# cliangyu/video-diffusion

Measured on AMD Instinct MI355X. Metric: denoise-steps/sec, higher is better.
Workload: dtype f32

## Files before the change

### include/vd_amd.h

```cpp
#ifndef VD_AMD_H
#define VD_AMD_H
#ifdef __cplusplus
extern "C" {
#endif

typedef struct vd_config {
    int image_size;
    int num_channels;
    int num_res_blocks;
    int num_heads;
    int T;
    int n_attention_ds;
    int attention_ds[8];
    int use_scale_shift_norm;
    int use_spatial_encoding;
    int use_frame_encoding;
    int enforce_position_invariance;
    int use_rpe_net;
    int allow_interactions_between_padding;
    float rp_alpha, rp_beta, rp_gamma;
    int time_embed_mult;
    int cond_emb_type;
    int learn_sigma;
} vd_config;
// ... 108 lines not shown
                  double* mse_out, void* stream);

int vd_window_begin(vd_engine* e, int B, int T, float* x, const float* obs_src, const float* obs_mask,
                    const float* latent_mask, const float* kinda_marg_mask, const long long* frame_indices,
                    int observed_frames, int sampler, int clip_denoised, float eta, unsigned long long seed,
                    unsigned long long offset, long long t_start, void* stream);
int vd_window_run(vd_engine* e, int n_steps, void* stream);
unsigned long long vd_window_generation(vd_engine* e);
int vd_window_graphs(vd_engine* e);

int vd_set_window_prefix_cache(vd_engine* e, int on);
int vd_window_prefix_frames(vd_engine* e);

int vd_set_window_suffix_skip(vd_engine* e, int on);
int vd_window_suffix_frames(vd_engine* e);

int vd_set_cfg_scale(vd_engine* e, float w);
float vd_cfg_scale(vd_engine* e);
int vd_op_cfg_combine(const float* out_c, const float* out_u, float w, long long n, float* out, void* stream);

int vd_set_guidance_rescale(vd_engine* e, float phi);
float vd_guidance_rescale(vd_engine* e);
int vd_set_dynamic_threshold(vd_engine* e, float p);
float vd_dynamic_threshold(vd_engine* e);
int vd_op_cfg_rescale(const float* out_c, const float* out_u, float w, const float* lat, int B, int T, long long frame_elems, float phi,
                      float* out, float* factor_out, void* stream);
int vd_op_dynamic_threshold(const float* x0, const float* lat, int B, int T, long long frame_elems, float p, float* out, float* s_out,
                            void* stream);

int vd_set_known_region(vd_engine* e, const float* known_src, const float* known_mask, const float* known_noise,
// ... 142 lines not shown
int vd_op_gn_bwd(const float* x0, const float* x1, int C0, int C, const float* affA, const float* affB, const float* mr,
                 const float* dy, int act, int nfr, int HW, const float* extra, float* dx0, int acc0, float* dx1, int acc1,
                 void* stream);
int vd_op_gn_temporal_bwd(const float* x, const float* gamma, const float* dy, int B, int T, int HW, int C, int accumulate,
                          float* dx, void* stream);
int vd_op_attn_temporal_bwd(const float* qkv, const float* Rk, const float* Rq, const float* Rv, const float* mask, int B,
                            int T, int HW, int C, int heads, int allow_pad, const float* dout, float* dqkv, void* stream);
int vd_op_attn_spatial_bwd(const float* qkv, int nfr, int L, int C, int heads, const float* dout, float* dqkv, void* stream);
int vd_op_out_conv_bwd(const float* deps, const float* w, int nfr, int H, int W, int C, int Cout, float* da, void* stream);
int vd_op_stem_col2im(const float* dcols, const float* obs, const float* lat, const float* km, int nfr, int H, int W,
                      int cond_mode, float* dx, void* stream);
int vd_op_sinus_embed(const float* t, int n, int dim, const float* freqs, float* out, void* stream);
int vd_op_frame_t(const long long* frame_indices, int B, int T, int center, float* tv, void* stream);
int vd_op_rpe_hidden(const float* te, int te_ld, const float* wbase, const long long* tab, const long long* frame_indices, int B, int T,
                     int C, float* E, int nz, long long zs_e, void* stream);
int vd_op_rpe_table(const float* table, const long long* frame_indices, int B, int T, int C, float alpha, float beta, float gamma,
                    float* R, void* stream);
int vd_op_posenc_add(const float* x, const float* P, const float* femb, int nfr, int HW, int C, float* y, void* stream);
int vd_op_assemble(const float* x, const float* obs_src, const float* obs_mask, const float* latent_mask, const float* kinda_marg_mask,
                   const float* t_model, int obs_t_mode, int B, int T, int H, int W, int Kpad, int cond_mode, const int* frame_list,
                   int n_list, int scalars_only, float* x_cols, float* t_frames, float* amask, void* stream);
int vd_op_move_rows(int scatter, const float* src, const int* list, int n, long long row_floats, float* dst, void* stream);
int vd_op_scatter_stats(const double* src, int split, int C, const int* list, int n, double* dst, void* stream);

typedef struct vd_lpips vd_lpips;
int vd_lpips_create(vd_lpips** out);
void vd_lpips_destroy(vd_lpips* h);
int vd_lpips_load_weight(vd_lpips* h, const char* name, const float* host, long long bytes);
long long vd_lpips_dim(int H, int W);
int vd_lpips_embed(vd_lpips* h, int N, int H, int W, const float* frames, float* out, void* stream);
// ... 28 lines not shown
```

### video-diffusion_amd/_lib.py

```python
import ctypes
import os
import subprocess

_HERE = os.path.dirname(os.path.abspath(__file__))
_CSRC = os.path.join(_HERE, "csrc")
SO_PATH = os.path.join(_HERE, "libvdamd.so")
SOURCES = ["igemm.hip", "conv_wino.hip", "conv_wino_r64.hip", "conv_wino_z128.hip", "gemm_frag.hip", "gemm_split.hip", "split_pack.hip", "norm.hip", "backward.hip", "attn_spatial.hip", "attn_temporal.hip", "attn_temporal_long.hip", "misc.hip", "guidance.hip", "known.hip", "measure.hip", "dps.hip", "ode_nll.hip", "engine.hip", "lpips.hip", "metrics.hip", "i3d.hip", "conv_cl.hip", "hallway.hip"]
HEADER = os.path.join(os.path.dirname(_HERE), "include", "vd_amd.h")
HEADERS = [os.path.join(_CSRC, "vd_common.h"), os.path.join(_CSRC, "wino_common.h"), os.path.join(_CSRC, "igemm_tile.h"), HEADER]
SOURCE_FLAGS = {"conv_wino_z128.hip": ["-mllvm", "-pragma-unroll-threshold=1000000"]}


def _toolchain():
    hipcc = os.environ.get("HIPCC", "/opt/rocm/bin/hipcc")
    flags = ["--offload-arch=gfx950", "-O3", "-std=c++17", "-fPIC", "-Wno-unused-value"] + \
        os.environ.get("VD_HIPCC_FLAGS", "").split()
    return hipcc, flags


def _sha(*parts):
    import hashlib
    h = hashlib.sha1()
    for p in parts:
        h.update(p if isinstance(p, bytes) else str(p).encode())
# ... 128 lines not shown
    "vd_dpmpp_2m_sde_sample": (_I, [_P, _I, _I, _P, _P, _P, _P, _P, _P, _P, _P, _I, _I, _P, _U, _U, _P, _P, _P, _P]),
    "vd_dpmpp_2m_sde_from_xstart": (_I, [_P, _I, _L, _P, _P, _P, _P, _I, _P, _U, _U, _P, _P, _P]),
    "vd_set_unipc_rows": (_I, [_P, _I, _P]),
    "vd_unipc_sample": (_I, [_P, _I, _I, _P, _P, _P, _P, _P, _P, _P, _P, _P, _P, _I, _I, _I, _P, _P, _P, _P, _P, _P, _P]),
    "vd_unipc_from_xstart": (_I, [_P, _I, _L, _P, _P, _P, _P, _P, _I, _P, _I, _P, _P, _P, _P, _P, _P]),
    "vd_p_mean_variance": (_I, [_P, _I, _I, _P, _P, _P, _P, _P, _P, _P, _I, _I, _P, _P, _P, _P]),
    "vd_vb_terms": (_I, [_P, _I, _I, _P, _P, _P, _P, _P, _I, _P, _P, _P, _P, _P, _P]),
    "vd_prior_bpd": (_I, [_P, _I, _I, _P, _P, _P, _P]),
    "vd_score_windows": (_I, [_P, _I, _I, _P, _P, _P, _P, _P, _P, _I, _U, _P, _P, _I, _P, _P]),
    "vd_op_eps_mse": (_I, [_P, _I, _I, _P, _P, _P, _I, _P, _U, _P, _P, _P, _P]),
    "vd_window_generation": (_U, [_P]),
    "vd_set_window_prefix_cache": (_I, [_P, _I]),
    "vd_window_prefix_frames": (_I, [_P]),
    "vd_set_window_suffix_skip": (_I, [_P, _I]),
    "vd_window_suffix_frames": (_I, [_P]),
    "vd_set_cfg_scale": (_I, [_P, _F]),
    "vd_cfg_scale": (_F, [_P]),
    "vd_op_cfg_combine": (_I, [_P, _P, _F, _L, _P, _P]),
    "vd_set_guidance_rescale": (_I, [_P, _F]),
    "vd_guidance_rescale": (_F, [_P]),
    "vd_set_dynamic_threshold": (_I, [_P, _F]),
    "vd_dynamic_threshold": (_F, [_P]),
    "vd_op_cfg_rescale": (_I, [_P, _P, _F, _P, _I, _I, _L, _F, _P, _P, _P]),
    "vd_op_dynamic_threshold": (_I, [_P, _P, _I, _I, _L, _F, _P, _P, _P]),
    "vd_set_known_region": (_I, [_P, _P, _P, _P, _U, _U]),
    "vd_known_region": (_I, [_P]),
    "vd_known_merge": (_I, [_P, _I, _I, _L, _P, _P, _P, _P, _P, _P, _U, _U, _P]),
    "vd_set_jump_rows": (_I, [_P, _I, _P, _P]),
    "vd_q_jump": (_I, [_P, _I, _I, _L, _P, _P, _P, _P, _U, _U, _P, _P]),
    "vd_window_jump": (_I, [_P, _I, _P]),
# ... 66 lines not shown
    "vd_igemm_variant_list": (_I, [ctypes.c_char_p, _I]),
    "vd_conv_wino_ksplit": (_I, [_I, _I, _I, _I]),
    "vd_op_conv_wino_split_k": (_I, [_P, _I, _I, _I, _I, _I, _P, _P, _P, _P, _I, _P, _I, _P, _I, _P]),
    "vd_op_linear_split_side": (_I, [_P, _P, _I, _I, _I, _I, _P, _P, _P, _P, _P, _P, _I, _P]),
    "vd_op_linear_batched": (_I, [_P, _I, _I, _I, _I, _P, _P, _P, _P]),
    "vd_op_out_conv": (_I, [_P, _P, _P, _P, _P, _I, _I, _I, _I, _I, _P, _P]),
    "vd_op_gn_bwd": (_I, [_P, _P, _I, _I, _P, _P, _P, _P, _I, _I, _I, _P, _P, _I, _P, _I, _P]),
    "vd_op_gn_temporal_bwd": (_I, [_P, _P, _P, _I, _I, _I, _I, _I, _P, _P]),
    "vd_op_attn_temporal_bwd": (_I, [_P, _P, _P, _P, _P, _I, _I, _I, _I, _I, _I, _P, _P, _P]),
    "vd_op_attn_spatial_bwd": (_I, [_P, _I, _I, _I, _I, _P, _P, _P]),
    "vd_op_out_conv_bwd": (_I, [_P, _P, _I, _I, _I, _I, _I, _P, _P]),
    "vd_op_stem_col2im": (_I, [_P, _P, _P, _P, _I, _I, _I, _I, _P, _P]),
    "vd_op_sinus_embed": (_I, [_P, _I, _I, _P, _P, _P]),
    "vd_op_frame_t": (_I, [_P, _I, _I, _I, _P, _P]),
    "vd_op_rpe_hidden": (_I, [_P, _I, _P, _P, _P, _I, _I, _I, _P, _I, _L, _P]),
    "vd_op_rpe_table": (_I, [_P, _P, _I, _I, _I, _F, _F, _F, _P, _P]),
    "vd_op_posenc_add": (_I, [_P, _P, _P, _I, _I, _I, _P, _P]),
    "vd_op_assemble": (_I, [_P, _P, _P, _P, _P, _P, _I, _I, _I, _I, _I, _I, _I, _P, _I, _I, _P, _P, _P, _P]),
    "vd_op_move_rows": (_I, [_I, _P, _P, _I, _L, _P, _P]),
    "vd_op_scatter_stats": (_I, [_P, _I, _I, _P, _I, _P, _P]),
    "vd_lpips_create": (_I, [ctypes.POINTER(_P)]),
    "vd_lpips_destroy": (None, [_P]),
    "vd_lpips_load_weight": (_I, [_P, ctypes.c_char_p, _P, _L]),
    "vd_lpips_dim": (_L, [_I, _I]),
    "vd_lpips_embed": (_I, [_P, _I, _I, _I, _P, _P, _P]),
    "vd_fps_select": (_I, [_I, _I, _L, _P, _I, _P, _I, _P, _P, _P]),
    "vd_frame_metrics": (_I, [_I, _I, _I, _I, _P, _P, _I, _D, _P, _P, _P]),
    "vd_pair_sqdist": (_I, [_I, _L, _P, _P, _P, _P]),
    "vd_i3d_create": (_I, [ctypes.POINTER(_P)]),
    "vd_i3d_destroy": (None, [_P]),
# ... 55 lines not shown
```

### video-diffusion_amd/csrc/engine.hip

```cpp
#include <cmath>
#include <cstring>
#include <unordered_map>
#include <vector>

#include "../../include/vd_amd.h"
#include "vd_common.h"

namespace vd {

thread_local std::string g_last_error;
void set_error(const std::string& msg) { g_last_error = msg; }

int launch_frame_t(const int64_t* fidx, int B, int T, int center, float* tv, hipStream_t s);

enum ParamKind { PK_RAW = 0, PK_CONV3, PK_STEM, PK_POSENC, PK_OUTCONV, PK_LINF, PK_CONV3W, PK_CONV3S,
                 PK_CONV3WU };

struct Param {
    std::string name;
    int nd = 0;
    long long shape[4] = {1, 1, 1, 1};
    size_t numel = 0;
    size_t packed = 0;
    size_t off = 0;
// ... 176 lines not shown
    int suf_blk = -2, suf_layer = -1;
    int p_posenc = -1, p_te0w, p_te0b, p_te2w, p_te2b, p_outgw, p_outgb, p_outw, p_outb;
    size_t film_w_off = 0, film_b_off = 0, te_w_off = 0, te_b_off = 0;
    int film_total = 0, te_total = 0;
    size_t packed_total = 0;
    float* wbuf = nullptr;
    bool wbuf_on_host = false;
    int put(void* dst, const void* src, size_t bytes) {
        if (wbuf_on_host) { std::memcpy(dst, src, bytes); return 0; }
        VD_HIP(hipMemcpy(dst, src, bytes, hipMemcpyHostToDevice));
        return 0;
    }
    struct RpeGroup { int C; std::vector<int> blocks; long long* d_hid = nullptr; long long* d_out = nullptr; };
    std::vector<RpeGroup> rpe_groups;
    std::vector<float*> rpe_R;
    int rpe_all(const float* te, const int64_t* fidx, int B, int T, hipStream_t st, Arena& ar);
    int rpe_tables();
    void rpe_group_blocks();
    float* d_freq_time = nullptr; int n_freq_time = 0;
    float* d_freq_frame = nullptr; int n_freq_frame = 0;
    float* d_tab = nullptr; int num_timesteps = 0;
    float* d_tmap = nullptr; float rescale = 1.f;
    float* d_w2m = nullptr;
    float* d_unipc = nullptr;
    float* d_jump = nullptr;
    char* ws = nullptr; size_t ws_cap = 0;
    bool ws_suf = false;
    int ws_B = 0, ws_T = 0; size_t ws_tail = 0;
    std::unordered_map<long long, size_t> ws_peaks;
    static size_t tm_bytes(int B) { return ((size_t)B * sizeof(float) + 255) & ~(size_t)255; }
    size_t out_floats(int B, int T) const { return (size_t)B * T * (cfg.learn_sigma ? 6 : 3) * cfg.image_size * cfg.image_size; }
// ... 664 lines not shown
            const RpeP* rp[3] = {&a.rq, &a.rk, &a.rv};
            for (int k = 0; k < 3; ++k) {
                const int z = 3 * (int)i + k;
                th[3 * z] = rp[k]->te_off; th[3 * z + 1] = (long long)params[rp[k]->dw].off; th[3 * z + 2] = (long long)params[rp[k]->db].off;
                to[2 * z] = (long long)params[rp[k]->ow].off; to[2 * z + 1] = (long long)params[rp[k]->ob].off;
            }
        }
        VD_HIP(hipMalloc(reinterpret_cast<void**>(&g.d_hid), th.size() * sizeof(long long)));
        VD_HIP(hipMalloc(reinterpret_cast<void**>(&g.d_out), to.size() * sizeof(long long)));
        VD_HIP(hipMemcpy(g.d_hid, th.data(), th.size() * sizeof(long long), hipMemcpyHostToDevice));
        VD_HIP(hipMemcpy(g.d_out, to.data(), to.size() * sizeof(long long), hipMemcpyHostToDevice));
    }
    return 0;
}

int vd_engine::rpe_all(const float* te, const int64_t* fidx, int B, int T, hipStream_t st, Arena& ar) {
    rpe_R.clear();
    if (!cfg.use_rpe_net || attn.empty() || !te_total) return 0;
    rpe_group_blocks();
    const size_t rrows = (size_t)B * T * T;
    rpe_R.assign(3 * attn.size(), nullptr);
    int rc = 0;
    for (auto& g : rpe_groups) {
        const int nn = 3 * (int)g.blocks.size(), C = g.C;
        float* Rg = ar.get<float>((size_t)nn * rrows * C);
        for (size_t i = 0; i < g.blocks.size(); ++i)
            for (int k = 0; k < 3; ++k) rpe_R[3 * g.blocks[i] + k] = Rg + (3 * i + k) * rrows * C;
        const size_t mk = ar.mark();
        float* Eh = ar.get<float>((size_t)nn * rrows * C);
        ar.release(mk);
        if (ar.dry) continue;
        VD_REQUIRE(g.d_hid && g.d_out, "rpe_all: offset tables missing (ensure_ws builds them)");
        if ((rc = launch_rpe_hidden_tab(te, te_total, wbuf, g.d_hid, fidx, B, T, C, Eh, nn, rrows * C, st))) return rc;
        IgemmArgs q = linear_args((int)rrows, C, C);
        q.src0 = Eh; q.out = Rg;
        q.wfrag = wbuf + params[attn[g.blocks[0]].rq.ow].off; q.bias = wbuf + params[attn[g.blocks[0]].rq.ob].off;
        q.zcount = nn; q.zs_a = q.zs_out = (int)(rrows * C); q.ztab = g.d_out; q.zbase = wbuf;
        if ((rc = igemm_p(q, st))) return rc;
    }
    return 0;
}

int vd_engine::forward(const FwdIn& in, hipStream_t st, Arena& ar, const PrefixPlan* pp, const SuffixPlan* sp) {
    const int B = in.B, T = in.T, N = B * T, S = cfg.image_size, mc = cfg.num_channels;
    int rc;
    VD_REQUIRE(!pp || (!tape && !ar.dry && pp->store && n_before_attn > 0), "prefix plan: executor steps only");
    VD_REQUIRE(!sp || (!tape && sp->n > 0 && sp->n <= N && (ar.dry || sp->list)), "suffix plan: executor steps only, at least one frame");
    struct SelGuard { ~SelGuard() { g_sel_nfr = 0; } } sel_guard;
    const int Npre = pp ? pp->n : N;
    float* x8 = ar.get<float>((size_t)Npre * S * S * STEM_KPAD);
    float* tfr = ar.get<float>(N);
    float* amask = ar.get<float>(N);
    float* tsin = ar.get<float>((size_t)N * mc);
// ... 12 lines not shown
            aa.frame_list = pp->list; aa.n_list = pp->n;
        }
        if ((rc = launch_assemble(aa, st))) return rc;
        if ((rc = launch_sinus_embed(tfr, N, mc, d_freq_time, tsin, st))) return rc;
        if ((rc = linear(tsin, N, mc, E, W(p_te0w), W(p_te0b), 0, nullptr, e1, st))) return rc;
        if ((rc = linear(e1, N, E, E, W(p_te2w), W(p_te2b), 1, nullptr, emb, st))) return rc;
        if ((rc = linear(emb, N, E, film_total, wbuf + film_w_off, wbuf + film_b_off, 1, nullptr, film, st))) return rc;
        if (te_total && (rc = linear(emb, N, E, te_total, wbuf + te_w_off, wbuf + te_b_off, 0, nullptr, te, st))) return rc;
        if (cfg.use_frame_encoding) {
            VD_REQUIRE(d_freq_frame && n_freq_frame == pos_ch / 2, "vd_set_freqs not called (frame frequencies)");
            if ((rc = launch_frame_t(in.fidx, B, T, cfg.enforce_position_invariance, ftv, st))) return rc;
            if ((rc = launch_sinus_embed(ftv, N, pos_ch, d_freq_frame, femb, st))) return rc;
        }
    }
    rpe_R.clear();
    if (!(pp && pp->build_only) && (rc = rpe_all(te, in.fidx, B, T, st, ar))) return rc;
    attn_seq = 0;
    std::vector<Tens> hs;
    Tens h{x8, STEM_KPAD, S};
    int Nrun = Npre;
    const float* film_full = film;
    if (pp || ar.dry) {
        float* fc = ar.get<float>((size_t)std::max(pp ? Npre : N, 1) * film_total);
        if (pp) {
            if ((rc = launch_gather_rows(film_full, pp->list, Npre, film_total, fc, st))) return rc;
            film = fc;
        }
    }
    auto run = [&](const std::vector<Layer>& blk, Tens in0, const Tens* in1, Tens* outp, size_t l0 = 0, size_t l1 = ~(size_t)0) -> int {
        const int N = Nrun;
        Tens cur = in0;
// ... 1242 lines not shown
    DynThreshArgs da{x0, nullptr, nullptr, nullptr, 0, lat, B, T, (long)frame_elems, p, out, s_out, nullptr, buf};
    return launch_dynamic_threshold(da, ws.st);
}

int vd_window_prefix_frames(vd_engine* e) {
    VD_REQUIRE(e, "null engine");
    return e->win_cur >= 0 && e->win_graphs[e->win_cur].store ? e->win_graphs[e->win_cur].n_inv : 0;
}

int vd_set_window_suffix_skip(vd_engine* e, int on) {
    VD_REQUIRE(e, "null engine");
    e->suffix_skip_on = on != 0;
    return 0;
}

int vd_window_suffix_frames(vd_engine* e) {
    VD_REQUIRE(e, "null engine");
    return e->win_cur >= 0 ? e->win_graphs[e->win_cur].n_suf : 0;
}

unsigned long long vd_window_generation(vd_engine* e) { return e ? e->win_gen : 0; }

int vd_window_run(vd_engine* e, int n_steps, void* stream) {
    VD_REQUIRE(e, "null engine");
    VD_REQUIRE(!e->win_lost, "window graphs invalidated (workspace growth or a new schedule since vd_window_begin): begin the window again");
    VD_REQUIRE(e->win_cur >= 0, "vd_window_begin first");
    const char* past = sampler_walks_up(e->win_graphs[e->win_cur].key.sampler) ? "more steps than the window has left (ddim_reverse_sample: t would pass num_timesteps - 1)"
                                                                  : "more steps than the window has left (t would pass 0)";
    VD_REQUIRE(n_steps >= 0 && n_steps <= e->win_left, past);
    hipStream_t st = static_cast<hipStream_t>(stream);
// ... 896 lines not shown
}

int vd_op_frame_t(const long long* fidx, int B, int T, int center, float* tv, void* stream) {
    VD_REQUIRE(fidx && tv && B > 0 && T > 0, "vd_op_frame_t: shape");
    return launch_frame_t(reinterpret_cast<const int64_t*>(fidx), B, T, center, tv, static_cast<hipStream_t>(stream));
}

int vd_op_rpe_hidden(const float* te, int te_ld, const float* wbase, const long long* tab, const long long* fidx, int B, int T, int C,
                     float* E, int nz, long long zs_e, void* stream) {
    VD_REQUIRE(te && wbase && tab && fidx && E && B > 0 && T > 0 && C > 0 && nz > 0, "vd_op_rpe_hidden: shape");
    VD_REQUIRE(te_ld >= C && zs_e >= (long long)B * T * T * C, "vd_op_rpe_hidden: te rows of at least C floats, a net's output inside its stride");
    return launch_rpe_hidden_tab(te, te_ld, wbase, tab, reinterpret_cast<const int64_t*>(fidx), B, T, C, E, nz, (size_t)zs_e,
                                 static_cast<hipStream_t>(stream));
}

int vd_op_rpe_table(const float* table, const long long* fidx, int B, int T, int C, float alpha, float beta, float gamma, float* R,
                    void* stream) {
    VD_REQUIRE(table && fidx && R && B > 0 && T > 0 && C > 0, "vd_op_rpe_table: shape");
    VD_REQUIRE(alpha >= 1.f && beta >= alpha && gamma >= alpha, "vd_op_rpe_table: bucket parameters 1 <= alpha <= beta, alpha <= gamma");
    return launch_rpe_table(table, reinterpret_cast<const int64_t*>(fidx), B, T, C, alpha, beta, gamma, R, static_cast<hipStream_t>(stream));
}

int vd_op_posenc_add(const float* x, const float* P, const float* femb, int nfr, int HW, int C, float* y, void* stream) {
    VD_REQUIRE(x && y && nfr > 0 && HW > 0 && C > 0 && C % 4 == 0, "vd_op_posenc_add: channels in 16-byte units");
    return launch_posenc_add(x, P, femb, nfr, HW, C, y, static_cast<hipStream_t>(stream));
}

int vd_op_assemble(const float* x, const float* obs_src, const float* obs_mask, const float* latent_mask, const float* kinda_marg_mask,
                   const float* t_model, int obs_t_mode, int B, int T, int H, int W, int Kpad, int cond_mode, const int* frame_list,
                   int n_list, int scalars_only, float* x_cols, float* t_frames, float* amask, void* stream) {
// ... 22 lines not shown
```

### video-diffusion_amd/csrc/gemm_frag.hip

```cpp
#include "vd_common.h"

namespace vd {

constexpr int GLD = 36;

#ifdef VD_GEMM_TIMING
__device__ unsigned long long g_gemm_stamp[6];
#define GEMM_STAMP(i) do { if (threadIdx.x == 0 && blockIdx.x == gridDim.x / 2 && blockIdx.y == 0) {                  \
        g_gemm_stamp[i] = __builtin_readcyclecounter();                                                             \
        if (i == 0) g_gemm_stamp[4] = __builtin_amdgcn_s_memrealtime();                                             \
        if (i == 3) g_gemm_stamp[5] = __builtin_amdgcn_s_memrealtime(); } } while (0)
extern "C" int vd_debug_gemm_stamps(unsigned long long* host_out) {
    return (int)hipMemcpyFromSymbol(host_out, HIP_SYMBOL(g_gemm_stamp), sizeof(g_gemm_stamp));
}
#else
#define GEMM_STAMP(i)
#endif

template <int BM, int BN, bool ACT>
__global__ __launch_bounds__(256, 3) void gemm_frag_kernel(IgemmArgs a) {
    constexpr int MI = BM / 64, NI = BN / 64, AR = BM / 32;
    extern __shared__ __attribute__((aligned(16))) float smem[];
    const int tid = threadIdx.x, lane = tid & 63, wave = __builtin_amdgcn_readfirstlane(tid >> 6);
    const int wm = wave >> 1, wn = wave & 1;
    const int lr = lane & 31, lh = lane >> 5;
    const int m0 = blockIdx.x * BM, n0 = blockIdx.y * BN;
    const int lrow = tid >> 3, lq = tid & 7;
    const int nchunk = a.Cin >> 5, ncoblk = a.Cout >> 5;
    const int C1 = a.Cin - a.C0;
    GEMM_STAMP(0);
    if (a.zcount > 1) {
        const int z = blockIdx.z;
        a.src0 += (size_t)z * a.zs_a; a.out += (size_t)z * a.zs_out;
        a.wfrag = a.zbase + a.ztab[2 * z];
        a.bias = a.zbase + a.ztab[2 * z + 1];
    }

    const auto asrc0 = __builtin_amdgcn_make_buffer_rsrc(const_cast<float*>(a.src0), 0, a.M * a.C0 * 4, 0x00020000);
    const auto asrc1 = __builtin_amdgcn_make_buffer_rsrc(const_cast<float*>(a.src1 ? a.src1 : a.src0), 0,
                                                         a.src1 ? a.M * C1 * 4 : 0, 0x00020000);
    unsigned ao0[AR], ao1[AR];
#pragma unroll
    for (int j = 0; j < AR; ++j) {
        const unsigned row = (unsigned)min(m0 + lrow + 32 * j, a.M - 1);
        ao0[j] = row * (unsigned)(a.C0 * 4) + lq * 16u;
        ao1[j] = row * (unsigned)(C1 * 4) + lq * 16u;
    }
    const auto bsrc = __builtin_amdgcn_make_buffer_rsrc(const_cast<float*>(a.wfrag), 0, a.Cin * a.Cout * 4, 0x00020000);
    unsigned bo[NI];
#pragma unroll
    for (int j = 0; j < NI; ++j) bo[j] = (unsigned)min((int)blockIdx.y * (BN / 32) + wn * NI + j, ncoblk - 1) * 4096u + lane * 16u;

    f32x4 ra[AR], bfr[4][NI], afr[2][MI];
    auto a_prefetch = [&](int chunk) {
        const int c = chunk * 32;
        if (c < a.C0) {
#pragma unroll
            for (int j = 0; j < AR; ++j)
                ra[j] = __builtin_bit_cast(f32x4, __builtin_amdgcn_raw_buffer_load_b128(asrc0, ao0[j], c * 4, 0));
        } else {
#pragma unroll
            for (int j = 0; j < AR; ++j)
                ra[j] = __builtin_bit_cast(f32x4, __builtin_amdgcn_raw_buffer_load_b128(asrc1, ao1[j], (c - a.C0) * 4, 0));
        }
    };
    auto a_store = [&](float* Ad) {
// ... 162 lines not shown
```

### video-diffusion_amd/csrc/gemm_split.hip

```cpp
#include <cstring>
#include <vector>

#include "vd_common.h"

namespace vd {

typedef __bf16 bf16x4 __attribute__((ext_vector_type(4)));
typedef __bf16 bf16x8 __attribute__((ext_vector_type(8)));
typedef unsigned u32x4 __attribute__((ext_vector_type(4)));
typedef unsigned u32x2 __attribute__((ext_vector_type(2)));

template <bool F16>
__device__ __forceinline__ f32x16 mfma_piece(u32x4 a, u32x4 b, f32x16 c) {
    if constexpr (F16) return __builtin_amdgcn_mfma_f32_32x32x16_f16(__builtin_bit_cast(f16x8, a), __builtin_bit_cast(f16x8, b), c, 0, 0, 0);
    else return __builtin_amdgcn_mfma_f32_32x32x16_bf16(__builtin_bit_cast(bf16x8, a), __builtin_bit_cast(bf16x8, b), c, 0, 0, 0);
}

#ifndef VD_GS_SKIP
#define VD_GS_SKIP 0
#endif
#ifdef VD_GS_TIMING
__device__ unsigned long long g_gs_stamp[8];
#define GS_STAMP(i) do { if (threadIdx.x == 0 && blockIdx.x == gridDim.x / 2 && blockIdx.y == 0) {                        \
        __builtin_amdgcn_sched_barrier(0); g_gs_stamp[i] = __builtin_amdgcn_s_memrealtime(); __builtin_amdgcn_sched_barrier(0); } } while (0)
// ... 23 lines not shown
template <int BM, int BN, bool ACT, bool CONV, bool F16 = true, bool SIDE = false>
__global__ __launch_bounds__(256, 2) void gemm_split_kernel(IgemmArgs a) {
    constexpr int MI = BM / 64, NI = BN / 64, AR = BM / 32;
    constexpr bool B2R = F16;
    constexpr int RING = NI >= 3 ? 2 : (BM == 64 && BN == 64) ? 6 : 3;
    constexpr int BP = B2R ? 2 : 3;
    constexpr int PF = BM == 64 ? 3 : 1;
    constexpr int NPL = F16 ? 2 : 3;
    constexpr int PLANE = BM * SROW, ABUF = NPL * PLANE;
    extern __shared__ __attribute__((aligned(16))) char smem_c[];
    const int tid = threadIdx.x, lane = tid & 63, wave = __builtin_amdgcn_readfirstlane(tid >> 6);
    GS_STAMP(0);
    const int wm = wave >> 1, wn = wave & 1;
    const int lr = lane & 31, lh = lane >> 5;
    int bxi = blockIdx.x, byi = blockIdx.y;
    if (gridDim.y > 1 && (gridDim.x & 7) == 0 && gridDim.x >= 128) {
        const unsigned lin = blockIdx.x + gridDim.x * blockIdx.y, xcd = lin & 7, loc = lin >> 3;
        byi = loc % gridDim.y;
        bxi = (loc / gridDim.y) * 8 + xcd;
    }
    const int m0 = bxi * BM, n0 = byi * BN;
    const int lgrp = tid >> 3, lrow = ((lgrp >> 1) & 3) + 8 * (lgrp >> 3) + 4 * (lgrp & 1), lq = tid & 7;
    const int cpt = a.Cin >> 5;
    const int nchunk = CONV ? 9 * cpt : cpt, ncoblk = a.Cout >> 5;
    const int C1 = a.Cin - a.C0;
    if (a.zcount > 1) {
        const int z = blockIdx.z;
        a.src0 += (size_t)z * a.zs_a; a.out += (size_t)z * a.zs_out;
        a.wfrag = a.zbase + a.ztab[2 * z];
        a.bias = a.zbase + a.ztab[2 * z + 1];
    }

    const auto asrc0 = __builtin_amdgcn_make_buffer_rsrc(const_cast<float*>(a.src0), 0,
                                                         (CONV ? a.nfr * a.Hs * a.Ws : a.M) * a.C0 * 4, 0x00020000);
    const auto asrc1 = __builtin_amdgcn_make_buffer_rsrc(const_cast<float*>(a.src1 ? a.src1 : a.src0), 0,
                                                         a.src1 ? a.M * C1 * 4 : 0, 0x00020000);
// ... 401 lines not shown
```

### video-diffusion_amd/csrc/igemm.hip

```cpp
#include <algorithm>

#include <string>

#include "igemm_tile.h"
#include "vd_common.h"

namespace vd {

constexpr int BK = IG_BK;
constexpr int LDP = IG_LDP;

template <int BM, int BN>
__global__ __launch_bounds__(256) void igemm_kernel(IgemmArgs a) {
    constexpr int MI = BM / 64, NI = BN / 64;
    constexpr int AR = BM / 32, BR = BN / 32;
    extern __shared__ __attribute__((aligned(16))) float smem[];
    float* As = smem;
    float* Bs = smem + 2 * BM * LDP;

    const int tid = threadIdx.x, lane = tid & 63, wave = tid >> 6;
    const int wm = wave >> 1, wn = wave & 1;
    const int lr = lane & 31;
    const int m0 = blockIdx.x * BM, n0 = blockIdx.y * BN;

// ... 119 lines not shown
    if (a.w == nullptr) { *why = "this shape runs on the generic kernel and needs [tap][Cout][Cin] weights"; return nullptr; }
    const int cls = tile >= 0 && tile <= 2 ? tile : 3;
    for (const IgemmRow& r : kIgemmRows)
        if (r.cls == cls) return &r;
    *why = "igemm.hip: no instantiation";
    return nullptr;
}

static const char* igemm_refusal(const IgemmArgs& a) {
    if (a.Cin % BK != 0) return "Cin must be a multiple of 32 (pad the operand)";
    if (!(a.C0 % BK == 0 && a.C0 <= a.Cin)) return "concat split must be a multiple of 32";
    if (!(a.src1 != nullptr || a.C0 == a.Cin)) return "second source missing";
    if (!(a.ksz == 1 || a.ksz == 3)) return "kernel size 1 or 3";
    if (!(a.M > 0 && a.Cout > 0)) return "empty problem";
    if (a.M != a.nfr * a.Ho * a.Wo) return "M != nfr*Ho*Wo";
    if (igemm_frames_per_launch(a) <= 0) return "one frame of this layer exceeds 2^28 elements";
    return nullptr;
}

static int igemm_one(const IgemmArgs& a, hipStream_t s, IgemmVariant* v) {
    const int tile = igemm_tile_class(igemm_sel_M(a), a.Cout);
    const char* why = nullptr;
    switch (igemm_kernel(a)) {
        case IK_R64_UPS:
            if (!conv_wino_r64_supported(a)) { why = "sub-pixel Upsample conv: shape not covered by conv_wino_r64.hip"; break; }
            return v ? (*v = conv_wino_r64_variant(a), 0) : launch_conv_wino_r64(a, s);
        case IK_SPLIT: return v ? (*v = gemm_split_variant(a, tile), 0) : launch_gemm_split(a, tile, s);
        case IK_Z128: return v ? (*v = conv_wino_z128_variant(a), 0) : launch_conv_wino_z128(a, s);
        case IK_R64: return v ? (*v = conv_wino_r64_variant(a), 0) : launch_conv_wino_r64(a, s);
        case IK_FRAG: return v ? (*v = gemm_frag_variant(a, tile), 0) : launch_gemm_frag(a, tile, s);
// ... 90 lines not shown
```

### video-diffusion_amd/csrc/misc.hip

```cpp
#include <algorithm>

#include "vd_common.h"

namespace vd {

__global__ __launch_bounds__(256) void assemble_kernel(AssembleArgs a) {
    const int n = a.frame_list ? a.frame_list[blockIdx.y] : blockIdx.y;
    const int HW = a.H * a.W;
    const float om = a.obs_mask[n], lm = a.lat_mask[n], km = a.km_mask[n];
    const float any = fminf(om + lm + km, 1.0f);
    const int Cs = a.cond_mode == 0 ? 5 : (a.cond_mode == 1 ? 6 : 3);
    if (blockIdx.x == 0 && threadIdx.x == 0 && !a.frame_list) {
        const float t = a.t_model[n / a.T];
        const float tobs = a.obs_t_mode == 0 ? 0.f : (a.obs_t_mode == 1 ? t : t - 1.f);
        float tf = t;
        if (a.cond_mode == 0) tf = tobs * om + t * (1.f - om);
        else if (a.cond_mode == 2) {
            bool any_obs = false;
            for (int k = 0; k < a.T; ++k) any_obs |= a.obs_mask[(n / a.T) * a.T + k] == 1.f;
            if (any_obs) tf = -1.f;
        }
        a.t_frames[n] = tf;
        a.amask[n] = any;
    }
// ... 118 lines not shown
        float s = 0.f;
        for (int t = 0; t < T; ++t) s += (float)fidx[b * T + t];
        mean = s / (float)T;
    }
    for (int t = threadIdx.x; t < T; t += blockDim.x) tv[b * T + t] = (float)fidx[b * T + t] - mean;
}

int launch_frame_t(const int64_t* fidx, int B, int T, int center, float* tv, hipStream_t s) {
    hipLaunchKernelGGL(frame_t_kernel, dim3(B), dim3(64), 0, s, fidx, T, center, tv);
    VD_HIP(hipGetLastError());
    return 0;
}

__global__ __launch_bounds__(256) void rpe_hidden_tab_kernel(const float* __restrict__ te, int te_ld, const float* __restrict__ wbase,
                                                             const long long* __restrict__ tab, const int64_t* __restrict__ fidx, int T, int C,
                                                             float* __restrict__ E, size_t zs_e) {
    __shared__ float feat[64][3];
    const long long* tz = tab + 3 * blockIdx.y;
    te += tz[0];
    const float* Wd = wbase + tz[1];
    const float* bd = wbase + tz[2];
    E += blockIdx.y * zs_e;
    const int bt = blockIdx.x, b = bt / T;
    for (int s0 = 0; s0 < T; s0 += 64) {
        const int ns = min(64, T - s0);
        __syncthreads();
        if ((int)threadIdx.x < ns) {
            const float d = (float)(fidx[bt] - fidx[b * T + s0 + threadIdx.x]);
            feat[threadIdx.x][0] = logf(1.0f + fmaxf(d, 0.f));
            feat[threadIdx.x][1] = logf(1.0f + fmaxf(-d, 0.f));
            feat[threadIdx.x][2] = d == 0.f ? 1.f : 0.f;
        }
        __syncthreads();
        for (int c = threadIdx.x; c < C; c += 256) {
            const float bc = bd[c], w0 = Wd[c * 3], w1 = Wd[c * 3 + 1], w2 = Wd[c * 3 + 2], tv = te[(size_t)bt * te_ld + c];
            for (int k = 0; k < ns; ++k) {
                const float lin = bc + feat[k][0] * w0 + feat[k][1] * w1 + feat[k][2] * w2;
                E[((size_t)bt * T + s0 + k) * C + c] = silu_f(tv + lin);
            }
        }
    }
}

int launch_rpe_hidden_tab(const float* te, int te_ld, const float* wbase, const long long* tab, const int64_t* fidx, int B, int T, int C,
                          float* E, int nz, size_t zs_e, hipStream_t s) {
    hipLaunchKernelGGL(rpe_hidden_tab_kernel, dim3(B * T, nz), dim3(256), 0, s, te, te_ld, wbase, tab, fidx, T, C, E, zs_e);
    VD_HIP(hipGetLastError());
    return 0;
}

__global__ __launch_bounds__(256) void rpe_table_kernel(const float* __restrict__ table, const int64_t* __restrict__ fidx,
                                                        int T, int C, float alpha, float beta, float gamma, double lg,
                                                        float* __restrict__ R) {
    const int row = blockIdx.x;
    const int s_ = row % T, bt = row / T, b = bt / T;
    const long long d = fidx[bt] - fidx[b * T + s_];
    long long id = d;
    const float ad = fabsf((float)d);
    if (ad > alpha) {
        double v = (double)alpha + log((double)ad / (double)alpha) / lg * ((double)beta - (double)alpha);
        const double r = rint(v);
// ... 757 lines not shown
```

### video-diffusion_amd/csrc/vd_common.h

```cpp
#pragma once
#include <hip/hip_runtime.h>
#include <cstdint>
#include <cstdio>
#include <string>
#include <vector>

typedef float f32x4 __attribute__((ext_vector_type(4)));
typedef float f32x16 __attribute__((ext_vector_type(16)));

namespace vd {

constexpr int kMaxWindowFrames = 128;
constexpr int kMaxGuidedWindowFrames = 32;

void set_error(const std::string& msg);
extern thread_local std::string g_last_error;

#define VD_HIP(call)                                                                   \
    do {                                                                               \
        hipError_t e_ = (call);                                                        \
        if (e_ != hipSuccess) {                                                        \
            vd::set_error(std::string(#call) + ": " + hipGetErrorString(e_));          \
            return -2;                                                                 \
        }                                                                              \
// ... 63 lines not shown
    const float* affA;
    const float* affB;
    int act;
    const float* res;
    int res_ld;
    const float* fbias;
    int fbias_ld;
    float* out;
    int ldo;
    int Cout, M;
    double* stats;
    int stats_split;
    int stats_hw;
    int zcount, zs_a, zs_out;
    const long long* ztab = nullptr; const float* zbase = nullptr;
    int wsplit;
    float* ksplit_ws;
    size_t ksplit_ws_floats;
};

struct AttnSpatialArgs {
    const float* qkv;
    float* out;
    int nfr, L, C, heads;
    float scale;
};

struct AttnTemporalArgs {
    const float* qkv;
    const float* Rk;
// ... 179 lines not shown
    int B, T, H, W, Kpad;
    int cond_mode;
    float* x_cols;
    float* t_frames;
    float* amask;
    const int* frame_list = nullptr;
    int n_list = 0;
    int scalars_only = 0;
};
int launch_assemble(const AssembleArgs& a, hipStream_t s);
int launch_gather_rows(const float* src, const int* list, int n, size_t row_floats, float* dst, hipStream_t s);
int launch_scatter_rows(const float* src, const int* list, int n, size_t row_floats, float* dst, hipStream_t s);
int launch_scatter_stats(const double* src, int split, int C, const int* list, int n, double* dst, hipStream_t s);
int launch_sinus_embed(const float* t, int n, int dim, const float* freqs, float* out, hipStream_t s);
int launch_rpe_hidden_tab(const float* te, int te_ld, const float* wbase, const long long* tab, const int64_t* fidx, int B, int T, int C,
                          float* E, int nz, size_t zs_e, hipStream_t s);
int launch_rpe_table(const float* table, const int64_t* fidx, int B, int T, int C, float alpha, float beta,
                     float gamma, float* R, hipStream_t s);
int launch_posenc_add(const float* x, const float* P, const float* femb, int nfr, int HW, int C, float* y,
                      hipStream_t s);
int launch_frame_t(const int64_t* fidx, int B, int T, int center, float* tv, hipStream_t s);
int launch_out_conv(const float* x, const float* affA, const float* affB, const float* w, const float* bias, int nfr,
                    int H, int W, int C, int Cout, float* out_nchw, hipStream_t s);

bool head_gemm_supported(int HW, int C, int ldt);
int launch_head_gemm(const float* h, const float* affA, const float* affB, const float* Wt, int nfr, int HW, int C, int ldt, float* T, hipStream_t s);
int launch_out_gather(const float* T, const float* bias, int nfr, int H, int W, int ldt, int Cout, float* out_nchw, hipStream_t s);

enum Sampler { SAMPLER_P = 0, SAMPLER_DDIM = 1, SAMPLER_DDIM_REVERSE = 2, SAMPLER_DPMPP_2M = 3, SAMPLER_DPMPP_2M_SDE = 4, SAMPLER_UNIPC = 5 };
inline bool sampler_valid(int s) { return s >= SAMPLER_P && s <= SAMPLER_UNIPC; }
inline bool sampler_walks_up(int s) { return s == SAMPLER_DDIM_REVERSE; }
// ... 280 lines not shown
```

Baseline: 51.21.

## Deduplicate RPE network computation across batch items with identical frame indices

```diff
diff --git a/include/vd_amd.h b/include/vd_amd.h
--- a/include/vd_amd.h
+++ b/include/vd_amd.h
@@ -146,6 +146,9 @@
 
 int vd_set_window_suffix_skip(vd_engine* e, int on);
 int vd_window_suffix_frames(vd_engine* e);
+
+int vd_set_rpe_dedup(vd_engine* e, int on);
+int vd_rpe_dedup(vd_engine* e);
 
 int vd_set_cfg_scale(vd_engine* e, float w);
 float vd_cfg_scale(vd_engine* e);
@@ -318,6 +321,7 @@
 int vd_op_frame_t(const long long* frame_indices, int B, int T, int center, float* tv, void* stream);
 int vd_op_rpe_hidden(const float* te, int te_ld, const float* wbase, const long long* tab, const long long* frame_indices, int B, int T,
                      int C, float* E, int nz, long long zs_e, void* stream);
+int vd_op_rpe_rep(const long long* frame_indices, const float* t_frames, int B, int T, int* rep, void* stream);
 int vd_op_rpe_table(const float* table, const long long* frame_indices, int B, int T, int C, float alpha, float beta, float gamma,
                     float* R, void* stream);
 int vd_op_posenc_add(const float* x, const float* P, const float* femb, int nfr, int HW, int C, float* y, void* stream);
diff --git a/video-diffusion_amd/_lib.py b/video-diffusion_amd/_lib.py
--- a/video-diffusion_amd/_lib.py
+++ b/video-diffusion_amd/_lib.py
@@ -166,6 +166,8 @@
     "vd_window_prefix_frames": (_I, [_P]),
     "vd_set_window_suffix_skip": (_I, [_P, _I]),
     "vd_window_suffix_frames": (_I, [_P]),
+    "vd_set_rpe_dedup": (_I, [_P, _I]),
+    "vd_rpe_dedup": (_I, [_P]),
     "vd_set_cfg_scale": (_I, [_P, _F]),
     "vd_cfg_scale": (_F, [_P]),
     "vd_op_cfg_combine": (_I, [_P, _P, _F, _L, _P, _P]),
@@ -262,6 +264,7 @@
     "vd_op_sinus_embed": (_I, [_P, _I, _I, _P, _P, _P]),
     "vd_op_frame_t": (_I, [_P, _I, _I, _I, _P, _P]),
     "vd_op_rpe_hidden": (_I, [_P, _I, _P, _P, _P, _I, _I, _I, _P, _I, _L, _P]),
+    "vd_op_rpe_rep": (_I, [_P, _P, _I, _I, _P, _P]),
     "vd_op_rpe_table": (_I, [_P, _P, _I, _I, _I, _F, _F, _F, _P, _P]),
     "vd_op_posenc_add": (_I, [_P, _P, _P, _I, _I, _I, _P, _P]),
     "vd_op_assemble": (_I, [_P, _P, _P, _P, _P, _P, _I, _I, _I, _I, _I, _I, _I, _P, _I, _I, _P, _P, _P, _P]),
diff --git a/video-diffusion_amd/csrc/engine.hip b/video-diffusion_amd/csrc/engine.hip
--- a/video-diffusion_amd/csrc/engine.hip
+++ b/video-diffusion_amd/csrc/engine.hip
@@ -214,7 +214,8 @@
     struct RpeGroup { int C; std::vector<int> blocks; long long* d_hid = nullptr; long long* d_out = nullptr; };
     std::vector<RpeGroup> rpe_groups;
     std::vector<float*> rpe_R;
-    int rpe_all(const float* te, const int64_t* fidx, int B, int T, hipStream_t st, Arena& ar);
+    int rpe_all(const float* te, const int64_t* fidx, const float* tfr, int B, int T, hipStream_t st, Arena& ar);
+    bool rpe_dedup = true;
     int rpe_tables();
     void rpe_group_blocks();
     float* d_freq_time = nullptr; int n_freq_time = 0;
@@ -909,13 +910,19 @@
     return 0;
 }
 
-int vd_engine::rpe_all(const float* te, const int64_t* fidx, int B, int T, hipStream_t st, Arena& ar) {
+int vd_engine::rpe_all(const float* te, const int64_t* fidx, const float* tfr, int B, int T, hipStream_t st, Arena& ar) {
     rpe_R.clear();
     if (!cfg.use_rpe_net || attn.empty() || !te_total) return 0;
     rpe_group_blocks();
     const size_t rrows = (size_t)B * T * T;
     rpe_R.assign(3 * attn.size(), nullptr);
     int rc = 0;
+    int* rep = B > 1 ? ar.get<int>(B) : nullptr;
+    if (!rpe_dedup) rep = nullptr;
+    if (rep && !ar.dry) {
+        ProfScope ps(PC_ELEMENTWISE, 0.0, 12.0 * B * T, st, "rpe_rep");
+        if ((rc = launch_rpe_rep(fidx, tfr, B, T, rep, st))) return rc;
+    }
     for (auto& g : rpe_groups) {
         const int nn = 3 * (int)g.blocks.size(), C = g.C;
         float* Rg = ar.get<float>((size_t)nn * rrows * C);
@@ -926,12 +933,17 @@
         ar.release(mk);
         if (ar.dry) continue;
         VD_REQUIRE(g.d_hid && g.d_out, "rpe_all: offset tables missing (ensure_ws builds them)");
-        if ((rc = launch_rpe_hidden_tab(te, te_total, wbuf, g.d_hid, fidx, B, T, C, Eh, nn, rrows * C, st))) return rc;
+        if ((rc = launch_rpe_hidden_tab(te, te_total, wbuf, g.d_hid, fidx, B, T, C, Eh, nn, rrows * C, st, rep))) return rc;
         IgemmArgs q = linear_args((int)rrows, C, C);
         q.src0 = Eh; q.out = Rg;
         q.wfrag = wbuf + params[attn[g.blocks[0]].rq.ow].off; q.bias = wbuf + params[attn[g.blocks[0]].rq.ob].off;
         q.zcount = nn; q.zs_a = q.zs_out = (int)(rrows * C); q.ztab = g.d_out; q.zbase = wbuf;
+        q.rep = rep; q.rep_rows = rep ? T * T : 0;
         if ((rc = igemm_p(q, st))) return rc;
+        if (rep) {
+            ProfScope ps(PC_ELEMENTWISE, 0.0, 8.0 * nn * (B - 1) * T * T * C, st, "rpe_replicate");
+            if ((rc = launch_rpe_replicate(Rg, rep, B, (size_t)T * T * C, nn, st))) return rc;
+        }
     }
     return 0;
 }
@@ -974,7 +986,7 @@
         }
     }
     rpe_R.clear();
-    if (!(pp && pp->build_only) && (rc = rpe_all(te, in.fidx, B, T, st, ar))) return rc;
+    if (!(pp && pp->build_only) && (rc = rpe_all(te, in.fidx, tfr, B, T, st, ar))) return rc;
     attn_seq = 0;
     std::vector<Tens> hs;
     Tens h{x8, STEM_KPAD, S};
@@ -2247,6 +2259,14 @@
     return 0;
 }
 
+int vd_set_rpe_dedup(vd_engine* e, int on) {
+    VD_REQUIRE(e, "null engine");
+    e->rpe_dedup = on != 0;
+    return 0;
+}
+
+int vd_rpe_dedup(vd_engine* e) { return e && e->rpe_dedup ? 1 : 0; }
+
 int vd_window_suffix_frames(vd_engine* e) {
     VD_REQUIRE(e, "null engine");
     return e->win_cur >= 0 ? e->win_graphs[e->win_cur].n_suf : 0;
@@ -3173,6 +3193,11 @@
                                  static_cast<hipStream_t>(stream));
 }
 
+int vd_op_rpe_rep(const long long* fidx, const float* t_frames, int B, int T, int* rep, void* stream) {
+    VD_REQUIRE(fidx && t_frames && rep && B > 0 && T > 0, "vd_op_rpe_rep: shape");
+    return launch_rpe_rep(reinterpret_cast<const int64_t*>(fidx), t_frames, B, T, rep, static_cast<hipStream_t>(stream));
+}
+
 int vd_op_rpe_table(const float* table, const long long* fidx, int B, int T, int C, float alpha, float beta, float gamma, float* R,
                     void* stream) {
     VD_REQUIRE(table && fidx && R && B > 0 && T > 0 && C > 0, "vd_op_rpe_table: shape");
diff --git a/video-diffusion_amd/csrc/gemm_frag.hip b/video-diffusion_amd/csrc/gemm_frag.hip
--- a/video-diffusion_amd/csrc/gemm_frag.hip
+++ b/video-diffusion_amd/csrc/gemm_frag.hip
@@ -24,7 +24,17 @@
     const int tid = threadIdx.x, lane = tid & 63, wave = __builtin_amdgcn_readfirstlane(tid >> 6);
     const int wm = wave >> 1, wn = wave & 1;
     const int lr = lane & 31, lh = lane >> 5;
-    const int m0 = blockIdx.x * BM, n0 = blockIdx.y * BN;
+    int bxi = blockIdx.x;
+    const int byi = blockIdx.y;
+    if (a.rep)
+        bxi = (blockIdx.x + blockIdx.y + gridDim.y * blockIdx.z) % gridDim.x;
+    const int m0 = bxi * BM, n0 = byi * BN;
+    if (a.rep) {
+        const int i1 = (min(m0 + BM, a.M) - 1) / a.rep_rows;
+        bool live = false;
+        for (int i = m0 / a.rep_rows; i <= i1; ++i) live |= a.rep[i] == i;
+        if (!live) return;
+    }
     const int lrow = tid >> 3, lq = tid & 7;
     const int nchunk = a.Cin >> 5, ncoblk = a.Cout >> 5;
     const int C1 = a.Cin - a.C0;
@@ -49,7 +59,7 @@
     const auto bsrc = __builtin_amdgcn_make_buffer_rsrc(const_cast<float*>(a.wfrag), 0, a.Cin * a.Cout * 4, 0x00020000);
     unsigned bo[NI];
 #pragma unroll
-    for (int j = 0; j < NI; ++j) bo[j] = (unsigned)min((int)blockIdx.y * (BN / 32) + wn * NI + j, ncoblk - 1) * 4096u + lane * 16u;
+    for (int j = 0; j < NI; ++j) bo[j] = (unsigned)min(byi * (BN / 32) + wn * NI + j, ncoblk - 1) * 4096u + lane * 16u;
 
     f32x4 ra[AR], bfr[4][NI], afr[2][MI];
     auto a_prefetch = [&](int chunk) {
diff --git a/video-diffusion_amd/csrc/gemm_split.hip b/video-diffusion_amd/csrc/gemm_split.hip
--- a/video-diffusion_amd/csrc/gemm_split.hip
+++ b/video-diffusion_amd/csrc/gemm_split.hip
@@ -61,12 +61,20 @@
     const int wm = wave >> 1, wn = wave & 1;
     const int lr = lane & 31, lh = lane >> 5;
     int bxi = blockIdx.x, byi = blockIdx.y;
-    if (gridDim.y > 1 && (gridDim.x & 7) == 0 && gridDim.x >= 128) {
+    if (a.rep) {
+        bxi = (blockIdx.x + blockIdx.y + gridDim.y * blockIdx.z) % gridDim.x;
+    } else if (gridDim.y > 1 && (gridDim.x & 7) == 0 && gridDim.x >= 128) {
         const unsigned lin = blockIdx.x + gridDim.x * blockIdx.y, xcd = lin & 7, loc = lin >> 3;
         byi = loc % gridDim.y;
         bxi = (loc / gridDim.y) * 8 + xcd;
     }
     const int m0 = bxi * BM, n0 = byi * BN;
+    if (a.rep) {
+        const int i1 = (min(m0 + BM, a.M) - 1) / a.rep_rows;
+        bool live = false;
+        for (int i = m0 / a.rep_rows; i <= i1; ++i) live |= a.rep[i] == i;
+        if (!live) return;
+    }
     const int lgrp = tid >> 3, lrow = ((lgrp >> 1) & 3) + 8 * (lgrp >> 3) + 4 * (lgrp & 1), lq = tid & 7;
     const int cpt = a.Cin >> 5;
     const int nchunk = CONV ? 9 * cpt : cpt, ncoblk = a.Cout >> 5;
diff --git a/video-diffusion_amd/csrc/igemm.hip b/video-diffusion_amd/csrc/igemm.hip
--- a/video-diffusion_amd/csrc/igemm.hip
+++ b/video-diffusion_amd/csrc/igemm.hip
@@ -157,6 +157,8 @@
     if (!(a.ksz == 1 || a.ksz == 3)) return "kernel size 1 or 3";
     if (!(a.M > 0 && a.Cout > 0)) return "empty problem";
     if (a.M != a.nfr * a.Ho * a.Wo) return "M != nfr*Ho*Wo";
+    if (a.rep && !(a.zcount > 1 && a.rep_rows > 0 && a.M % a.rep_rows == 0))
+        return "representative table: a batched launch over rows of whole batch items";
     if (igemm_frames_per_launch(a) <= 0) return "one frame of this layer exceeds 2^28 elements";
     return nullptr;
 }
diff --git a/video-diffusion_amd/csrc/misc.hip b/video-diffusion_amd/csrc/misc.hip
--- a/video-diffusion_amd/csrc/misc.hip
+++ b/video-diffusion_amd/csrc/misc.hip
@@ -156,8 +156,9 @@
 
 __global__ __launch_bounds__(256) void rpe_hidden_tab_kernel(const float* __restrict__ te, int te_ld, const float* __restrict__ wbase,
                                                              const long long* __restrict__ tab, const int64_t* __restrict__ fidx, int T, int C,
-                                                             float* __restrict__ E, size_t zs_e) {
+                                                             float* __restrict__ E, size_t zs_e, const int* __restrict__ rep) {
     __shared__ float feat[64][3];
+    if (rep && rep[blockIdx.x / T] != (int)(blockIdx.x / T)) return;
     const long long* tz = tab + 3 * blockIdx.y;
     te += tz[0];
     const float* Wd = wbase + tz[1];
@@ -185,8 +186,50 @@
 }
 
 int launch_rpe_hidden_tab(const float* te, int te_ld, const float* wbase, const long long* tab, const int64_t* fidx, int B, int T, int C,
-                          float* E, int nz, size_t zs_e, hipStream_t s) {
-    hipLaunchKernelGGL(rpe_hidden_tab_kernel, dim3(B * T, nz), dim3(256), 0, s, te, te_ld, wbase, tab, fidx, T, C, E, zs_e);
+                          float* E, int nz, size_t zs_e, hipStream_t s, const int* rep) {
+    hipLaunchKernelGGL(rpe_hidden_tab_kernel, dim3(B * T, nz), dim3(256), 0, s, te, te_ld, wbase, tab, fidx, T, C, E, zs_e, rep);
+    VD_HIP(hipGetLastError());
+    return 0;
+}
+
+__global__ __launch_bounds__(64) void rpe_rep_kernel(const int64_t* __restrict__ fidx, const float* __restrict__ tfr, int T, int* __restrict__ rep) {
+    __shared__ int best;
+    const int b = blockIdx.x;
+    if (threadIdx.x == 0) best = b;
+    __syncthreads();
+    for (int c = threadIdx.x; c < b; c += 64) {
+        bool diff = false;
+        for (int t = 0; t < T; ++t)
+            diff |= fidx[(size_t)c * T + t] != fidx[(size_t)b * T + t] ||
+                    __float_as_uint(tfr[(size_t)c * T + t]) != __float_as_uint(tfr[(size_t)b * T + t]);
+        if (!diff) atomicMin(&best, c);
+    }
+    __syncthreads();
+    if (threadIdx.x == 0) rep[b] = best;
+}
+
+int launch_rpe_rep(const int64_t* fidx, const float* tfr, int B, int T, int* rep, hipStream_t s) {
+    hipLaunchKernelGGL(rpe_rep_kernel, dim3(B), dim3(64), 0, s, fidx, tfr, T, rep);
+    VD_HIP(hipGetLastError());
+    return 0;
+}
+
+__global__ __launch_bounds__(256) void rpe_replicate_kernel(float* __restrict__ R, const int* __restrict__ rep, size_t item_q, size_t net_q) {
+    const int b = blockIdx.y, r = rep[b];
+    if (r == b) return;
+    f32x4* net = reinterpret_cast<f32x4*>(R) + blockIdx.z * net_q;
+    const f32x4* src = net + (size_t)r * item_q;
+    f32x4* dst = net + (size_t)b * item_q;
+#pragma unroll 4
+    for (size_t i = (size_t)blockIdx.x * 256 + threadIdx.x; i < item_q; i += (size_t)gridDim.x * 256) dst[i] = src[i];
+}
+
+int launch_rpe_replicate(float* R, const int* rep, int B, size_t item_floats, int nz, hipStream_t s) {
+    VD_REQUIRE(item_floats % 4 == 0 && (reinterpret_cast<uintptr_t>(R) & 15) == 0, "rpe_replicate: items of whole 16-byte units");
+    VD_REQUIRE(B <= 65535 && nz <= 65535, "rpe_replicate: grid limits");
+    const size_t item_q = item_floats / 4;
+    const unsigned chunks = (unsigned)std::min<size_t>(std::max<size_t>((item_q + 2047) / 2048, 1), 1024);
+    hipLaunchKernelGGL(rpe_replicate_kernel, dim3(chunks, B, nz), dim3(256), 0, s, R, rep, item_q, item_q * B);
     VD_HIP(hipGetLastError());
     return 0;
 }
diff --git a/video-diffusion_amd/csrc/vd_common.h b/video-diffusion_amd/csrc/vd_common.h
--- a/video-diffusion_amd/csrc/vd_common.h
+++ b/video-diffusion_amd/csrc/vd_common.h
@@ -101,6 +101,7 @@
     int stats_hw;
     int zcount, zs_a, zs_out;
     const long long* ztab = nullptr; const float* zbase = nullptr;
+    const int* rep = nullptr; int rep_rows = 0;
     int wsplit;
     float* ksplit_ws;
     size_t ksplit_ws_floats;
@@ -310,7 +311,9 @@
 int launch_scatter_stats(const double* src, int split, int C, const int* list, int n, double* dst, hipStream_t s);
 int launch_sinus_embed(const float* t, int n, int dim, const float* freqs, float* out, hipStream_t s);
 int launch_rpe_hidden_tab(const float* te, int te_ld, const float* wbase, const long long* tab, const int64_t* fidx, int B, int T, int C,
-                          float* E, int nz, size_t zs_e, hipStream_t s);
+                          float* E, int nz, size_t zs_e, hipStream_t s, const int* rep = nullptr);
+int launch_rpe_rep(const int64_t* fidx, const float* tfr, int B, int T, int* rep, hipStream_t s);
+int launch_rpe_replicate(float* R, const int* rep, int B, size_t item_floats, int nz, hipStream_t s);
 int launch_rpe_table(const float* table, const int64_t* fidx, int B, int T, int C, float alpha, float beta,
                      float gamma, float* R, hipStream_t s);
 int launch_posenc_add(const float* x, const float* P, const float* femb, int nfr, int HW, int C, float* y,
```

After: 51.43, median of 6. No clear change (+0.4%).
